# beltegeuse/rustlight

Measured on AMD Instinct MI355X. Metric: Msamples/s (paths/s) at 1080p x 128spp cbox, higher is better.
Workload: dtype f32

## Files before the change

rustlight_amd/csrc/device_types.h:

```cpp
#pragma once
#include <stdint.h>

namespace rl {

struct alignas(16) BvhNode {
    float lmin[3]; float lmax0;
    float lmax12[2]; float rmin01[2];
    float rmin2; float rmax[3];
    int32_t left, right; int32_t pad0, pad1;
};
static_assert(sizeof(BvhNode) == 64, "BvhNode must be 64 bytes");
static const int32_t RL_CHILD_NONE = (int32_t)0x80000000;

struct alignas(16) BvhNode2 {
    float lox[4], loy[4], loz[4];
    float hix[4], hiy[4], hiz[4];
    int32_t slot[4];
    int32_t child[2];
    int32_t pad[2];
};
static_assert(sizeof(BvhNode2) == 128, "BvhNode2 must be 128 bytes");

struct alignas(16) Bvh4Node {
    float org[3];
// ... 6 lines not shown
static_assert(sizeof(Bvh4Node) == 64, "Bvh4Node must be 64 bytes");

struct alignas(16) TriRecord {
    float v0[3]; float n0;
    float e1[3]; float n1;
    float e2[3]; float n2;
    float det;
    int32_t mesh;
    int32_t tri;
    int32_t gtri;
};
static_assert(sizeof(TriRecord) == 64, "TriRecord must be 64 bytes");

struct ColorTex {
    int32_t type;
    float c0[3];
    float c1[3];
    float offset[2];
    float scale[2];
    float line_width;
    int32_t bitmap;
    int32_t pad[3];
};
static_assert(sizeof(ColorTex) == 64, "ColorTex must be 64 bytes");

struct BitmapDesc { uint32_t w, h; uint64_t offset; };

struct Material {
    int32_t type;
    int32_t distribution;
    float exponent, weight_specular;
    float alpha_u, alpha_v;
    float glass_eta, glass_inv_eta;
    int32_t smooth;
    int32_t twosided;
    int32_t pad[2];
    ColorTex diffuse, specular, transmittance, eta, k;
};

struct MeshRecord {
    int32_t material;
    int32_t flags;
    float emission[3];
    float inv_area;
    float emitter_pdf;
    uint32_t vertex_base;
    uint32_t tri_base;
    uint32_t n_tris;
    uint32_t cdf_base;
    uint32_t ats_base;
    int32_t emission_type;
    float emission_scale;
    int32_t emission_bitmap;
};
enum { MESH_HAS_NORMALS = 1, MESH_HAS_UV = 2, MESH_IS_LIGHT = 4 };

enum { EMITTER_MESH = 0, EMITTER_ENV = 1, EMITTER_POINT = 2, EMITTER_DIRECTIONAL = 3 };
struct EmitterRecord {
    int32_t kind;
    int32_t mesh;
    float v[3];
    float c[3];
    float center[3];
    float radius;
    float pad[4];
};
static_assert(sizeof(EmitterRecord) == 64, "EmitterRecord must be 64 bytes");

struct LightNode {
    float bmin[3], bmax[3];
    float axis[3];
    float phi, cos_theta_o, cos_theta_e;
    int32_t left, right, parent;
    int32_t light;
};
static_assert(sizeof(LightNode) == 64, "LightNode must be 64 bytes");

struct CameraRecord {
    float sample_to_camera[16];
    float to_world[16];
    float position[3];
    uint32_t width, height;
};

struct MediumRecord {
    int32_t enabled;
    float sigma_a[3], sigma_s[3], sigma_t[3];
    int32_t phase;
    float g;
};

struct DeviceScene {
    const BvhNode* nodes;
    const TriRecord* tris;
    float root_min[3], root_max[3];
    int32_t root;
    uint32_t n_nodes, n_prims;
    uint32_t stack_depth;
    const BvhNode* nodes_t;
    int32_t root_t;
    const BvhNode2* nodes2;
    const Bvh4Node* nodes4;
    int32_t root4;
    uint32_t stack_depth4;
    const uint32_t* tri_indices;
    const float* positions;
    const float* normals;
    const float* uvs;
    const MeshRecord* meshes;
    const Material* materials;
    const BitmapDesc* bitmaps;
    const float* bitmap_texels;
    const EmitterRecord* emitters;
    const float* emitters_cdf;
    uint32_t n_emitters;
    int32_t env_emitter;
    float env_color[3];
    float env_pdf;
    uint32_t env_w, env_h;
    const float* env_texels;
    const float* env_cond_cdf;
    const float* env_cond_func;
    const float* env_marg_cdf;
    float env_marg_func_int;
    float env_sel_pdf;
    int32_t ats_root;
    const LightNode* ats_nodes;
    const int32_t* ats_light_mesh;
    const int32_t* ats_light_prim;
    const uint32_t* ats_leaf_of;
    const float* mesh_cdf;
    uint32_t n_meshes;
    CameraRecord camera;
    MediumRecord medium;
};

}
```

rustlight_amd/csrc/host/scene.cpp:

```cpp
#include "scene.h"
#include "../kernels/wavefront.h"
#include "../detmath_shared.h"

#include <algorithm>
#include <cmath>
#include <cstring>

namespace rl {

static const float kEpsilon = 0.0001f;
static const float kPi = 3.14159265358979323846f;

void build_cdf(const std::vector<float>& elements, std::vector<float>* cdf, float* func_int) {
    cdf->clear();
    cdf->reserve(elements.size() + 1);
    float cur = 0.0f;
    const float n = (float)elements.size();
    for (float e : elements) {
        cdf->push_back(cur);
        cur += e / n;
    }
    cdf->push_back(cur);
    if (cur != 0.0f)
        for (float& x : *cdf) x /= cur;
// ... 6 lines not shown
    t->type = d.type;
    for (int i = 0; i < 3; i++) { t->c0[i] = d.color0[i]; t->c1[i] = d.color1[i]; }
    for (int i = 0; i < 2; i++) { t->offset[i] = d.offset[i]; t->scale[i] = d.scale[i]; }
    t->line_width = d.line_width;
    t->bitmap = d.bitmap_id;
}

static Material convert_material(const rl_bsdf_desc& b) {
    Material m;
    std::memset(&m, 0, sizeof(m));
    m.type = b.type;
    m.distribution = b.distribution;
    m.exponent = b.exponent;
    m.weight_specular = b.weight_specular;
    m.alpha_u = b.alpha_u;
    m.alpha_v = b.alpha_v;
    m.glass_eta = b.glass_eta;
    m.glass_inv_eta = 1.0f / b.glass_eta;
    bool delta = false;
    switch (b.type) {
        case RL_BSDF_METAL: delta = b.distribution == RL_MICROFACET_NONE; break;
        case RL_BSDF_GLASS: delta = true; break;
        case RL_BSDF_SUBSTRATE: delta = b.distribution == RL_MICROFACET_NONE; break;
        default: break;
    }
    m.smooth = delta ? 1 : 0;
    m.twosided = b.type == RL_BSDF_GLASS ? 0 : 1;
    convert_color(b.diffuse, &m.diffuse);
    convert_color(b.specular, &m.specular);
    convert_color(b.transmittance, &m.transmittance);
    convert_color(b.eta, &m.eta);
    convert_color(b.k, &m.k);
    return m;
}

void flatten_scene(const rl_scene& scene, FlatScene* out) {
    *out = FlatScene();
    uint32_t vbase = 0, tbase = 0;
    for (size_t mi = 0; mi < scene.meshes.size(); mi++) {
        const HostMesh& m = scene.meshes[mi];
        MeshRecord r;
        std::memset(&r, 0, sizeof(r));
        r.material = (int32_t)out->materials.size();
        out->materials.push_back(convert_material(m.bsdf));
        r.flags = (m.normals.empty() ? 0 : MESH_HAS_NORMALS) | (m.uvs.empty() ? 0 : MESH_HAS_UV) | (m.is_light ? MESH_IS_LIGHT : 0);
        for (int i = 0; i < 3; i++) r.emission[i] = m.emission[i];
        r.emission_type = m.emission_type; r.emission_scale = m.emission_scale; r.emission_bitmap = m.emission_bitmap;
        r.inv_area = 1.0f / m.area_total();
        r.emitter_pdf = 0.0f;
        r.vertex_base = vbase;
        r.tri_base = tbase;
        r.n_tris = (uint32_t)m.n_tris();
        r.cdf_base = (uint32_t)out->mesh_cdf.size();
        out->mesh_tri_base.push_back(tbase);
        out->mesh_cdf.insert(out->mesh_cdf.end(), m.cdf.begin(), m.cdf.end());
        for (size_t v = 0; v < m.positions.size(); v++) {
            out->positions.push_back(m.positions[v].x); out->positions.push_back(m.positions[v].y); out->positions.push_back(m.positions[v].z);
            Vec3 n = m.normals.empty() ? Vec3{0, 0, 0} : m.normals[v];
            out->normals.push_back(n.x); out->normals.push_back(n.y); out->normals.push_back(n.z);
            out->uvs.push_back(m.uvs.empty() ? 0.0f : m.uvs[2 * v]);
            out->uvs.push_back(m.uvs.empty() ? 0.0f : m.uvs[2 * v + 1]);
        }
        for (uint32_t i : m.indices) out->tri_indices.push_back(i + vbase);
        vbase += (uint32_t)m.positions.size();
        tbase += (uint32_t)m.n_tris();
        out->meshes.push_back(r);
    }
    for (size_t e = 0; e < scene.emitters.size(); e++)
        if (scene.emitters[e].kind == EMITTER_MESH)
            out->meshes[scene.emitters[e].mesh].emitter_pdf = scene.emitters_cdf[e + 1] - scene.emitters_cdf[e];
    uint64_t off = 0;
    for (const HostBitmap& b : scene.bitmaps) {
        out->bitmaps.push_back({b.w, b.h, off});
        out->bitmap_texels.insert(out->bitmap_texels.end(), b.rgb.begin(), b.rgb.end());
        off += (uint64_t)b.w * b.h;
    }
}

}

using namespace rl;

bool rl_scene::rebuild_camera() {
    if (!to_world.inverse(&to_local)) return false;
    const float x_v = flip ? 1.0f : -1.0f;
    const float aspect = (float)width / (float)height;
    const float fov_rad = fov_axis == 0 ? fov_degrees * kPi / 180.0f : fov_degrees * aspect * kPi / 180.0f;
    camera_to_sample = Mat4::scale(-0.5f, -0.5f * aspect, 1.0f)
                                .times(Mat4::translate(-1.0f, -1.0f / aspect, 0.0f))
                                .times(perspective(fov_rad, 1.0f, 1e-2f, 1000.0f))
                                .times(Mat4::scale(x_v, 1.0f, -1.0f));
    if (!camera_to_sample.inverse(&sample_to_camera)) return false;
    cam_pos = to_world.xform_point({0.0f, 0.0f, 0.0f});
    has_camera = true;
    return true;
}

extern "C" {

int rl_scene_create(rl_scene** out) {
    if (!out) return RL_ERR_INVALID_ARGUMENT;
    *out = new rl_scene();
    return RL_OK;
}
void rl_scene_destroy(rl_scene* scene) { delete scene; }

// ... 372 lines not shown
```

rustlight_amd/csrc/host/scene.h:

```cpp
#pragma once
#include <cstdint>
#include <string>
#include <vector>

#include "../../../include/rustlight_amd.h"
#include "../device_types.h"
#include "hostmath.h"

namespace rl {

struct HostMesh {
    std::vector<Vec3> positions;
    std::vector<uint32_t> indices;
    std::vector<Vec3> normals;
    std::vector<float> uvs;
    rl_bsdf_desc bsdf;
    bool is_light = false;
    float emission[3] = {0, 0, 0};
    int emission_type = 0;
    float emission_scale = 1.0f;
    int emission_bitmap = -1;
    std::vector<float> cdf;
    float func_int = 0.0f;
    size_t n_tris() const { return indices.size() / 3; }
// ... 15 lines not shown
    rl::Vec3 cam_pos{0, 0, 0};
    std::vector<rl::HostMesh> meshes;
    std::vector<rl::HostBitmap> bitmaps;
    rl::MediumRecord medium{};
    bool emitters_built = false;
    std::vector<rl::EmitterRecord> other_emitters;
    bool has_env = false; float env_color[3] = {0, 0, 0};
    rl::HostBitmap env_map{0, 0, {}};
    std::vector<float> env_cond_cdf, env_cond_func, env_marg_cdf;
    float env_marg_func_int = 0.0f;
    std::vector<rl::EmitterRecord> emitters;
    std::vector<float> emitters_cdf;
    float bsphere_center[3] = {0, 0, 0};
    float bsphere_radius = 0;
    bool want_ats = false;
    int32_t ats_root = -1;
    std::vector<rl::LightNode> ats_nodes;
    std::vector<int32_t> ats_light_emitter, ats_light_prim;
    std::vector<uint32_t> ats_leaf_of;
    std::vector<uint32_t> ats_emitter_base;

    bool rebuild_camera();
};

namespace rl {

void build_cdf(const std::vector<float>& elements, std::vector<float>* cdf, float* func_int);

struct BvhBuild {
    std::vector<BvhNode> nodes;
    std::vector<TriRecord> tris;
    float root_min[3], root_max[3];
    int32_t root = RL_CHILD_NONE;
    uint32_t stack_depth = 1;
    std::vector<float> ref_boxes;
    std::vector<uint64_t> ref_info, ref_count;
    std::vector<int32_t> ref_prim_mesh, ref_prim_tri;
};
void build_bvh(const rl_scene& scene, BvhBuild* out);
void treelet_blocks(const BvhBuild& bvh, std::vector<BvhNode>* nodes_out, int32_t* root_out);
void two_level_nodes(const BvhBuild& bvh, std::vector<BvhNode2>* out, uint64_t* stats3 = nullptr);
struct Bvh4Build { std::vector<Bvh4Node> nodes; int32_t root = RL_CHILD_NONE; uint32_t stack_depth = 1; };
void build_bvh4(const BvhBuild& bvh, Bvh4Build* out);

struct FlatScene {
    std::vector<uint32_t> tri_indices;
    std::vector<float> positions, normals, uvs;
    std::vector<MeshRecord> meshes;
    std::vector<Material> materials;
    std::vector<BitmapDesc> bitmaps;
    std::vector<float> bitmap_texels;
    std::vector<float> mesh_cdf;
    std::vector<uint32_t> mesh_tri_base;
};
void flatten_scene(const rl_scene& scene, FlatScene* out);

int build_light_tree(rl_scene* scene, std::string* err);
int host_math_sweep(int fn, uint32_t first_bits, uint32_t stride, uint32_t period, size_t n, const float* b, size_t n_b, int swap, float* out);
int read_pfm(const char* path, uint32_t* w, uint32_t* h, std::vector<float>* rgb);
int load_pbrt(const char* path, bool use_shading_normals, rl_scene** out, std::string* err);

}
```

rustlight_amd/csrc/kernels/shading.hip.h:

```cpp
#pragma once
#include "../device_types.h"
#include "devmath.hip.h"

namespace rl {

enum { BSDF_DIFFUSE = 0, BSDF_PHONG = 1, BSDF_METAL = 2, BSDF_GLASS = 3, BSDF_SUBSTRATE = 4 };
enum { TEXTURE_CONSTANT = 0, TEXTURE_CHECKER = 1, TEXTURE_GRID = 2, TEXTURE_BITMAP = 3 };
enum { MICRO_NONE = 0, MICRO_BECKMANN = 1, MICRO_GGX = 2 };
enum { PDF_SOLID_ANGLE = 0, PDF_AREA = 1, PDF_DISCRETE = 2 };

struct SurfacePoint {
    V3 p, n_g, n_s, wi;
    Frame frame;
    V2 uv;
    bool has_uv;
    int mesh;
};

RL_DEV unsigned long long f32_as_usize(float f) { if (!(f > 0.0f)) return 0ull; if (f >= 1.8446744e19f) return ~0ull; return (unsigned long long)f; }
RL_DEV int f32_as_i32(float f) { if (f != f) return 0; if (f >= 2147483648.0f) return 2147483647; if (f <= -2147483648.0f) return (-2147483647 - 1); return (int)f; }
RL_DEV float modulo1(float a) { return fmodf(fmodf(a, 1.0f) + 1.0f, 1.0f); }

RL_DEV Col tex_color(const DeviceScene& sc, const ColorTex& t, bool has_uv, V2 uv) {
    if (t.type == TEXTURE_CONSTANT) return mkc(t.c0[0], t.c0[1], t.c0[2]);
// ... 401 lines not shown
    unsigned long long x = f32_as_usize(ux * (float)sc.env_w), y = f32_as_usize(uy * (float)sc.env_h);
    unsigned long long i = (unsigned long long)sc.env_w * y + x;
    if (i >= (unsigned long long)sc.env_w * sc.env_h) return czero();
    return mkc(sc.env_texels[3 * i], sc.env_texels[3 * i + 1], sc.env_texels[3 * i + 2]);
}
RL_DEV float env_direct_pdf(const DeviceScene& sc, V3 d) {
    if (sc.env_w == 0u) return sc.env_pdf;
    V2 uv = env_to_spherical(d);
    float p = env_bin_pdf(sc, f32_as_usize(uv.x * (float)sc.env_w), f32_as_usize(uv.y * (float)sc.env_h));
    float st = m_sinf(kPi * uv.y);
    float v = st == 0.0f ? 0.0f : div_rn(p, (2.0f * powi_f(kPi, 2)) * st);
    return v * sc.env_sel_pdf;
}
RL_DEV void env_sample_direction(const DeviceScene& sc, V2 u, V3* d, Col* value, float* pdf) {
    float y = cdf_sample_continuous(sc.env_marg_cdf, sc.env_h, u.y);
    unsigned long long row = f32_as_usize(y);
    float x = cdf_sample_continuous(sc.env_cond_cdf + row * (sc.env_w + 1u), sc.env_w, u.x);
    x = clamp_f(x, 0.0f, (float)sc.env_w - 1.0f);
    y = clamp_f(y, 0.0f, (float)sc.env_h - 1.0f);
    unsigned long long px = f32_as_usize(x), py = f32_as_usize(y);
    const float* t = sc.env_texels + 3ull * (py * sc.env_w + px);
    float p = env_bin_pdf(sc, px, py);
    float sp, cp, st, ct;
    m_sincosf(div_rn(2.0f * kPi, (float)sc.env_w) * x, &sp, &cp);
    m_sincosf(div_rn(kPi, (float)sc.env_h) * y, &st, &ct);
    *d = mk3(st * cp, st * sp, ct);
    if (st == 0.0f) { *value = czero(); *pdf = 0.0f; }
    else { *value = mkc(t[0], t[1], t[2]); *pdf = div_rn(p, (2.0f * powi_f(kPi, 2)) * st); }
}

RL_DEV bool bsphere_intersect(V3 center, float radius, V3 o, V3 d, float tnear, float tfar, float* t_out) {
    V3 d_p = center - o;
    float a = length2(d);
    float b = 2.0f * dot(d_p, d);
    float c = length2(d_p) - radius * radius;
    float x0, x1;
    if (a == 0.0f) {
        if (b == 0.0f) return false;
        float v = div_rn(-c, b);
        x0 = v; x1 = v;
    } else {
        float disc = b * b - 4.0f * a * c;
        if (disc < 0.0f) return false;
        float d_sqrt = sqrt_rn(disc);
        float tmp = b < 0.0f ? -0.5f * (b - d_sqrt) : -0.5f * (b + d_sqrt);
        float r0 = div_rn(tmp, a), r1 = div_rn(c, tmp);
        if (r0 > r1) { x0 = r1; x1 = r0; } else { x0 = r0; x1 = r1; }
    }
    if (x0 < tnear) { if (x1 < tfar) { *t_out = x1; return true; } return false; }
    if (x0 < tfar) { *t_out = x0; return true; }
    return false;
}

template <int LIGHTS = LIGHTS_ANY>
RL_DEV void mesh_sample_triangle(const DeviceScene& sc, const MeshRecord& mr, unsigned int prim, float pdf_area, V3 p, V2 uv, LightSample* ls) {
    unsigned int gtri = mr.tri_base + prim;
    unsigned int i0 = sc.tri_indices[3 * gtri], i1 = sc.tri_indices[3 * gtri + 1], i2 = sc.tri_indices[3 * gtri + 2];
    V3 v0 = mk3(sc.positions[3 * i0], sc.positions[3 * i0 + 1], sc.positions[3 * i0 + 2]);
    V3 v1 = mk3(sc.positions[3 * i1], sc.positions[3 * i1 + 1], sc.positions[3 * i1 + 2]);
    V3 v2 = mk3(sc.positions[3 * i2], sc.positions[3 * i2 + 1], sc.positions[3 * i2 + 2]);
    V2 b = uniform_sample_triangle(uv);
    float w2 = 1.0f - b.x - b.y;
    V3 pos = v0 * b.x + v1 * b.y + v2 * w2;
    V3 n_g = normalize(cross(v2 - v0, v1 - v0));
    if (mr.flags & MESH_HAS_NORMALS) {
        V3 n0 = mk3(sc.normals[3 * i0], sc.normals[3 * i0 + 1], sc.normals[3 * i0 + 2]);
        V3 n1 = mk3(sc.normals[3 * i1], sc.normals[3 * i1 + 1], sc.normals[3 * i1 + 2]);
        V3 n2 = mk3(sc.normals[3 * i2], sc.normals[3 * i2 + 1], sc.normals[3 * i2 + 2]);
        V3 n = n0 * b.x + n1 * b.y + n2 * w2;
        float nl = length2(n);
        if (nl == 0.0f) n = n_g;
        else if (nl != 1.0f) n = n / sqrt_rn(nl);
        if (dot(n_g, n) < 0.0f) n_g = -n_g;
    }
    if (pdf_area < 0.0f) pdf_area = div_rn(1.0f, length(cross(v1 - v0, v2 - v0)) * 0.5f);
    V3 d = pos - p;
    float dist = length(d);
    if (dist != 0.0f) d = d / dist;
    float geom = dist != 0.0f ? div_rn(rmax(dot(n_g, -d), 0.0f), dist * dist) : 0.0f;
    float pdf = geom == 0.0f ? 0.0f : div_rn(pdf_area, geom);
    Col emit;
    if (LIGHTS == LIGHTS_AREA_ONLY || __builtin_expect(mr.emission_type == 0, 1)) emit = mkc(mr.emission[0], mr.emission[1], mr.emission[2]);
    else emit = mesh_emit_sampled(sc.bitmaps, sc.bitmap_texels, sc.uvs, mr.emission_type, mr.emission_scale, mr.emission_bitmap, (mr.flags & MESH_HAS_UV) != 0, i0, i1, i2, b.x, b.y, w2);
    ls->weight = pdf == 0.0f ? czero() : emit * geom / pdf_area;
    ls->pdf = pdf; ls->pdf_kind = PDF_SOLID_ANGLE;
    ls->p = pos; ls->n = n_g; ls->d = d;
}

RL_DEV float ats_cos_subtended(V3 bmin, V3 bmax, V3 p) {
    V3 c = (bmax - bmin) * 0.5f + bmin;
    float radius = length(c - bmax);
    if (length2(p - c) < radius * radius) return -1.0f;
    float sin2 = div_rn(radius * radius, length2(c - p));
    return sqrt_rn(rmax(1.0f - sin2, 0.0f));
}
RL_DEV float ats_cos_sub(float sa, float ca, float sb, float cb) { return ca > cb ? 1.0f : ca * cb + sa * sb; }
RL_DEV float ats_sin_sub(float sa, float ca, float sb, float cb) { return ca > cb ? 1.0f : sa * cb - ca * sb; }
RL_DEV float ats_importance(const LightNode& nd, V3 p, bool has_n, V3 n) {
    V3 bmin = mk3(nd.bmin[0], nd.bmin[1], nd.bmin[2]), bmax = mk3(nd.bmax[0], nd.bmax[1], nd.bmax[2]);
    V3 pc = (bmax - bmin) * 0.5f + bmin;
    float d2 = rmax(length2(p - pc), 0.0001f);
    V3 wi = normalize(p - pc);
    float cos_theta = dot(mk3(nd.axis[0], nd.axis[1], nd.axis[2]), wi);
    float sin_theta = sqrt_rn(rmax(1.0f - cos_theta * cos_theta, 0.0f));
    float cos_u = ats_cos_subtended(bmin, bmax, p);
    float sin_u = sqrt_rn(rmax(1.0f - cos_u * cos_u, 0.0f));
    float sin_o = sqrt_rn(rmax(1.0f - nd.cos_theta_o * nd.cos_theta_o, 0.0f));
    float cos_x = ats_cos_sub(sin_theta, cos_theta, sin_o, nd.cos_theta_o);
    float sin_x = ats_sin_sub(sin_theta, cos_theta, sin_o, nd.cos_theta_o);
    float cos_p = ats_cos_sub(sin_x, cos_x, sin_u, cos_u);
    if (cos_p <= nd.cos_theta_e) return 0.0f;
    float imp = div_rn(nd.phi * cos_p, d2);
    if (has_n) {
        float cos_i = fabsf(dot(wi, n));
        float sin_i = sqrt_rn(rmax(1.0f - cos_i * cos_i, 0.0f));
        imp = imp * ats_cos_sub(sin_i, cos_i, sin_u, cos_u);
    }
// ... 159 lines not shown
```

rustlight_amd/csrc/kernels/trace.hip.h:

```cpp
#pragma once
#include "../device_types.h"
#include "devmath.hip.h"
#include <type_traits>

namespace rl {

struct Hit { float t, u, v; int prim; int steps = 0, tris = 0, fetches = 0; };

#ifndef RL_LDS_NODE_STRIDE
#define RL_LDS_NODE_STRIDE 17
#endif
#ifndef RL_LDS_TRI_STRIDE4
#define RL_LDS_TRI_STRIDE4 5
#endif
static constexpr int kLdsNodeStride = RL_LDS_NODE_STRIDE;
static constexpr int kLdsTriStride4 = RL_LDS_TRI_STRIDE4;
RL_DEV __host__ unsigned lds_nodes_float4s(unsigned n_nodes) { return (n_nodes * (unsigned)kLdsNodeStride + 3u) / 4u; }
RL_DEV __host__ unsigned lds_scene_float4s(unsigned n_nodes, unsigned n_prims) { return lds_nodes_float4s(n_nodes) + n_prims * (unsigned)kLdsTriStride4; }

RL_DEV bool slab(V3 lo, V3 hi, V3 o, V3 inv_d, float tnear, float tfar, float* t_entry) {
    const float x0 = (lo.x - o.x) * inv_d.x, x1 = (hi.x - o.x) * inv_d.x;
    const float y0 = (lo.y - o.y) * inv_d.y, y1 = (hi.y - o.y) * inv_d.y;
    const float z0 = (lo.z - o.z) * inv_d.z, z1 = (hi.z - o.z) * inv_d.z;
    const bool sx = inv_d.x < 0.0f, sy = inv_d.y < 0.0f, sz = inv_d.z < 0.0f;
// ... 21 lines not shown
        const V3 pv = (o + t * d) - v0;
        const V3 u0 = cross(e1, pv);
        const V3 w0 = cross(pv, e2);
        const bool facing = !(dot(u0, n) < 0.0f) & !(dot(w0, n) < 0.0f);
        const float uu = dot(u0, u0), ww = dot(w0, w0);
#if defined(RL_FAST_MATH)
        accept = facing & (det > 0.0f) & (__builtin_amdgcn_sqrtf(uu) + __builtin_amdgcn_sqrtf(ww) <= det);
#else
        const float s = __builtin_amdgcn_sqrtf(uu) + __builtin_amdgcn_sqrtf(ww);
        const bool in_range = __builtin_fminf(__builtin_fminf(uu, ww), det) >= 0x1p-100f;
        const bool sure_in = in_range & (s <= det * 0.99999f), sure_out = in_range & (s >= det * 1.00001f);
        accept = facing & sure_in;
        if (facing & !sure_in & !sure_out) {
            const float v = div_rn(sqrt_rn(uu), det);
            const float u = div_rn(sqrt_rn(ww), det);
            accept = !(u < 0.0f || v < 0.0f || u > 1.0f || v > 1.0f) && (u + v <= 1.0f);
        }
#endif
    }
    hit.t = accept ? t : hit.t;
    hit.prim = accept ? prim : hit.prim;
    return accept;
}

struct SceneRecs {
    const float4* nodes;
    const float4* tris;
};

struct NodeFetchLds;
struct NodeFetchGlobal;
template <bool LDS_ONLY>
struct TravStackT {
    using NodeFetch = typename std::conditional<LDS_ONLY, NodeFetchLds, NodeFetchGlobal>::type;
    static constexpr bool kLdsOnly = LDS_ONLY;
#ifdef RL_FAST_MATH
    static constexpr bool kBvh4 = !LDS_ONLY;
#else
    static constexpr bool kBvh4 = false;
#endif
    static constexpr bool kTwoLevel = false;
    static constexpr int kTriStride4 = LDS_ONLY ? kLdsTriStride4 : 4;
    static constexpr int kNodeRefScale = LDS_ONLY ? 4 * kLdsNodeStride : 1;
    static constexpr int lds_stride = 256;
    typedef int i2v __attribute__((ext_vector_type(2)));
    typedef __attribute__((address_space(3))) i2v LdsPair;
    typedef __attribute__((address_space(1))) i2v GlobPair;
    using LdsPtr = typename std::conditional<kBvh4, int2*, LdsPair*>::type;
    using GlobPtr = typename std::conditional<kBvh4, int*, GlobPair*>::type;
    LdsPtr lds; int lds_levels;
    GlobPtr glob; size_t glob_stride;
    RL_DEV void push(int sp, int code, float dist, bool counts = true) const { push_to(lds, glob, sp, code, dist, counts); }
    RL_DEV void get(int sp, int* code, float* dist) const { get_from(lds, glob, sp, code, dist); }
    RL_DEV void push_to(LdsPair* l, GlobPair* g, int sp, int code, float dist, bool counts) const {
        i2v e; e.x = code; e.y = __float_as_int(dist);
        if (LDS_ONLY || sp < lds_levels) l[sp * lds_stride] = e;
        else if (counts) g[(size_t)(sp - lds_levels) * glob_stride] = e;
    }
    RL_DEV void get_from(const LdsPair* l, const GlobPair* g, int sp, int* code, float* dist) const {
        i2v e;
        if (LDS_ONLY || sp < lds_levels) e = l[sp * lds_stride];
        else e = g[(size_t)(sp - lds_levels) * glob_stride];
        *code = e.x; *dist = __int_as_float(e.y);
    }
    RL_DEV void push_to(int2* l, int* g, int sp, int code, float dist, bool) const {
        if (sp < lds_levels) l[sp * lds_stride] = make_int2(code, __float_as_int(dist));
        else { size_t k = (size_t)(2 * (sp - lds_levels)); g[k * glob_stride] = code; g[(k + 1) * glob_stride] = __float_as_int(dist); }
    }
    RL_DEV void get_from(const int2* l, const int* g, int sp, int* code, float* dist) const {
        if (sp < lds_levels) { const int2 e = l[sp * lds_stride]; *code = e.x; *dist = __int_as_float(e.y); }
        else { size_t k = (size_t)(2 * (sp - lds_levels)); *code = g[k * glob_stride]; *dist = __int_as_float(g[(k + 1) * glob_stride]); }
    }
};
using TravStack = TravStackT<false>;
struct TravStack2 : TravStackT<false> {
    static constexpr bool kTwoLevel = true;
    static constexpr bool kBvh4 = false;
    RL_DEV explicit TravStack2(const TravStackT<false>& s) : TravStackT<false>(s) {}
};

typedef float f4v __attribute__((ext_vector_type(4)));
typedef const f4v __attribute__((address_space(4))) F4c;
struct NodePlanes { float lnx, lny, lnz, lfx, lfy, lfz, rnx, rny, rnz, rfx, rfy, rfz; int id1, id2; };

struct NodeFetchLds {
    static constexpr bool kHasUniform = false;
    RL_DEV NodePlanes uniform(int) const { return NodePlanes(); }
    const float *nx, *ny, *nz, *fx, *fy, *fz; const int* ids;
    RL_DEV NodeFetchLds(const SceneRecs& recs, V3 inv_d) {
        const float* b = reinterpret_cast<const float*>(recs.nodes);
        const bool sx = inv_d.x < 0.0f, sy = inv_d.y < 0.0f, sz = inv_d.z < 0.0f;
        nx = b + (sx ? 3 : 0); fx = b + (sx ? 0 : 3);
        ny = b + (sy ? 4 : 1); fy = b + (sy ? 1 : 4);
        nz = b + (sz ? 5 : 2); fz = b + (sz ? 2 : 5);
        ids = reinterpret_cast<const int*>(b) + 12;
    }
    RL_DEV NodePlanes operator()(int cur) const {
        NodePlanes p;
#define RL_AT(ptr, off) (*reinterpret_cast<const float*>(reinterpret_cast<const char*>(ptr) + cur + 4 * (off)))
        p.lnx = RL_AT(nx, 0); p.rnx = RL_AT(nx, 6); p.lny = RL_AT(ny, 0); p.rny = RL_AT(ny, 6); p.lnz = RL_AT(nz, 0); p.rnz = RL_AT(nz, 6);
        p.lfx = RL_AT(fx, 0); p.rfx = RL_AT(fx, 6); p.lfy = RL_AT(fy, 0); p.rfy = RL_AT(fy, 6); p.lfz = RL_AT(fz, 0); p.rfz = RL_AT(fz, 6);
        p.id1 = __float_as_int(RL_AT(ids, 0)); p.id2 = __float_as_int(RL_AT(ids, 1));
#undef RL_AT
        return p;
    }
};
// ... 2 lines not shown
    RL_DEV NodeFetchGlobal(const SceneRecs& recs, V3 inv_d) : nodes(recs.nodes), sx(inv_d.x < 0.0f), sy(inv_d.y < 0.0f), sz(inv_d.z < 0.0f) {}
    RL_DEV NodePlanes operator()(int cur) const {
        const float4* q = nodes + 4 * cur;
        const float4 a = q[0], b = q[1], c = q[2];
        const float4 e = q[3];
        NodePlanes p;
        p.lnx = sx ? a.w : a.x; p.lfx = sx ? a.x : a.w; p.lny = sy ? b.x : a.y; p.lfy = sy ? a.y : b.x; p.lnz = sz ? b.y : a.z; p.lfz = sz ? a.z : b.y;
        p.rnx = sx ? c.y : b.z; p.rfx = sx ? b.z : c.y; p.rny = sy ? c.z : b.w; p.rfy = sy ? b.w : c.z; p.rnz = sz ? c.w : c.x; p.rfz = sz ? c.x : c.w;
        p.id1 = __float_as_int(e.x); p.id2 = __float_as_int(e.y);
        return p;
    }
    static constexpr bool kHasUniform = true;
    RL_DEV NodePlanes uniform(int cur) const {
        const F4c* q = (const F4c*)(nodes) + 4 * cur;
        const f4v a = q[0], b = q[1], c = q[2], e = q[3];
        NodePlanes p;
        p.lnx = sx ? a.w : a.x; p.lfx = sx ? a.x : a.w; p.lny = sy ? b.x : a.y; p.lfy = sy ? a.y : b.x; p.lnz = sz ? b.y : a.z; p.lfz = sz ? a.z : b.y;
        p.rnx = sx ? c.y : b.z; p.rfx = sx ? b.z : c.y; p.rny = sy ? c.z : b.w; p.rfy = sy ? b.w : c.z; p.rnz = sz ? c.w : c.x; p.rfz = sz ? c.x : c.w;
        p.id1 = __float_as_int(e.x); p.id2 = __float_as_int(e.y);
        return p;
    }
};

#ifndef RL_VOTE_NUM
#define RL_VOTE_NUM 3
#define RL_VOTE_DEN 2
#endif
#ifndef RL_VOTE4_NUM
#define RL_VOTE4_NUM 3
#define RL_VOTE4_DEN 2
#endif
template <bool ANY_HIT, class Stack>
RL_DEV bool traverse4(const SceneRecs& recs, int root, V3 root_lo, V3 root_hi, V3 o, V3 d, float tnear, float tfar, Hit& hit, const Stack& st);
template <bool ANY_HIT, class Stack>
RL_DEV bool traverse2(const SceneRecs& recs, int root, V3 root_lo, V3 root_hi, V3 o, V3 d, float tnear, float tfar, Hit& hit, const Stack& st);
template <class Stack>
RL_DEV const float4* streamed_nodes(const DeviceScene& sc) {
    return Stack::kBvh4 ? reinterpret_cast<const float4*>(sc.nodes4) : (Stack::kTwoLevel ? reinterpret_cast<const float4*>(sc.nodes2) : reinterpret_cast<const float4*>(sc.nodes));
}

template <bool ANY_HIT, class Stack>
RL_DEV bool traverse(const SceneRecs& recs, int root, V3 root_lo, V3 root_hi, V3 o, V3 d, float tnear, float tfar,
                     Hit& hit, const Stack& st) {
    if constexpr (Stack::kBvh4) return traverse4<ANY_HIT>(recs, root, root_lo, root_hi, o, d, tnear, tfar, hit, st);
    if constexpr (Stack::kTwoLevel) return traverse2<ANY_HIT>(recs, root, root_lo, root_hi, o, d, tnear, tfar, hit, st);
    V3 inv_d = mk3(div_rn(1.0f, d.x), div_rn(1.0f, d.y), div_rn(1.0f, d.z));
    float dummy;
    int cur = root >= 0 ? root * Stack::kNodeRefScale : root;
    if (!slab(root_lo, root_hi, o, inv_d, tnear, tfar, &dummy)) cur = RL_CHILD_NONE;
    int sp = 0;
    bool found = false;
    typename Stack::NodeFetch fetch(recs, inv_d);
    constexpr int kPop = -1;
    auto node_trip = [&]() {
        if (cur >= 0) {
            hit.steps++;
            NodePlanes p;
            const int cur0 = __builtin_amdgcn_readfirstlane(cur);
            if (Stack::NodeFetch::kHasUniform && __ballot(cur != cur0) == 0ull) p = fetch.uniform(cur0);
            else p = fetch(cur);
            const float d1 = __builtin_fmaxf(__builtin_fmaxf(__builtin_fmaxf((p.lnx - o.x) * inv_d.x, (p.lny - o.y) * inv_d.y), (p.lnz - o.z) * inv_d.z), tnear);
            const float f1 = __builtin_fminf(__builtin_fminf(__builtin_fminf((p.lfx - o.x) * inv_d.x, (p.lfy - o.y) * inv_d.y), (p.lfz - o.z) * inv_d.z), hit.t);
            const float d2 = __builtin_fmaxf(__builtin_fmaxf(__builtin_fmaxf((p.rnx - o.x) * inv_d.x, (p.rny - o.y) * inv_d.y), (p.rnz - o.z) * inv_d.z), tnear);
            const float f2 = __builtin_fminf(__builtin_fminf(__builtin_fminf((p.rfx - o.x) * inv_d.x, (p.rfy - o.y) * inv_d.y), (p.rfz - o.z) * inv_d.z), hit.t);
            const bool v1 = !(f1 <= d1), v2 = !(f2 <= d2);
            const bool right_first = v2 & (!v1 | (d1 > d2));
            st.push(sp, right_first ? p.id1 : p.id2, right_first ? d1 : d2, v1 && v2);
            sp += (v1 && v2) ? 1 : 0;
            cur = (v1 || v2) ? (right_first ? p.id2 : p.id1) : kPop;
        }
        if (cur == kPop) {
            cur = RL_CHILD_NONE;
            if (sp > 0) {
                sp--;
                int code; float dist;
                st.get(sp, &code, &dist);
                cur = dist < hit.t ? code : kPop;
            }
        }
    };
    auto leaf_visit = [&]() -> bool {
        const unsigned int code = (unsigned int)(~cur);
        const int first = (int)(code >> 2), count = (int)(code & 3u);
        bool uni = false;
        if (Stack::NodeFetch::kHasUniform) uni = __ballot(cur != __builtin_amdgcn_readfirstlane(cur)) == 0ull;
        for (int k = 0; k < count; k++) {
            hit.tris++;
            float4 q0, q1, q2, q3;
            if (uni) {
                const F4c* q = (const F4c*)(recs.tris) + 4 * (__builtin_amdgcn_readfirstlane(first) + k);
                const f4v a = q[0], b = q[1], c = q[2], e = q[3];
                q0 = make_float4(a.x, a.y, a.z, a.w); q1 = make_float4(b.x, b.y, b.z, b.w); q2 = make_float4(c.x, c.y, c.z, c.w); q3 = make_float4(e.x, e.y, e.z, e.w);
            } else {
                const float4* q = recs.tris + Stack::kTriStride4 * (first + k);
                q0 = q[0]; q1 = q[1]; q2 = q[2]; q3 = q[3];
            }
            if (tri_test(q0, q1, q2, q3, o, d, hit, first + k)) {
                found = true;
                if (ANY_HIT) return true;
            }
        }
        cur = kPop;
        return false;
    };
    if (Stack::kLdsOnly) {
        while (cur != RL_CHILD_NONE) {
            while (cur >= 0 || cur == kPop) node_trip();
            if (cur != RL_CHILD_NONE && leaf_visit()) return true;
        }
    } else {
#if defined(RL_TRAVERSE_SPARSE)
        while (cur != RL_CHILD_NONE) {
            if (cur >= 0 || cur == kPop) node_trip();
            else if (leaf_visit()) return true;
        }
#else
        for (;;) {
            const bool in_node = cur >= 0 || cur == kPop;
            const bool in_leaf = !in_node && cur != RL_CHILD_NONE;
            const int n_node = __popcll(__ballot(in_node)), n_leaf = __popcll(__ballot(in_leaf));
            if (n_node + n_leaf == 0) break;
            if (n_node > 0 && n_node * RL_VOTE_DEN >= RL_VOTE_NUM * n_leaf) { if (in_node) node_trip(); }
            else if (in_leaf && leaf_visit()) return true;
        }
#endif
    }
    if (!ANY_HIT && found) {
        const float4* q = recs.tris + Stack::kTriStride4 * hit.prim;
        tri_uv(q[0], q[1], q[2], q[3], o, d, hit.t, &hit.u, &hit.v);
    }
// ... 448 lines not shown
```

rustlight_amd/csrc/kernels/wavefront.hip:

```cpp
#include <hip/hip_runtime.h>

#include <algorithm>
#include <atomic>
#include <chrono>
#include <cmath>
#include <cstdio>
#include <cstring>
#include <memory>
#include <string>
#include <thread>
#include <vector>

#include "common.hip.h"
#include "rngjump.h"
#include "../host/hip_buffer.h"
#include "../host/photontree.h"
#include "../host/beamtree.h"
#include "phototree.h"
#include "../host/scene.h"
#include "wavefront.h"
#include "knobs.h"
#include "light.hip.h"

namespace rl {
// ... 109 lines not shown
template <bool LDS_SCENE>
__global__ void __launch_bounds__(256) k_shadow(RenderConst rc, DeviceScene sc, Pool pool, StackConf stc) { trace_kernel_body<LDS_SCENE, true>(sc, pool, stc); }

__global__ void __launch_bounds__(256) k_trace_batch(DeviceScene sc, StackConf stc, unsigned n, const float* o, const float* d, float* t_out, float* u_out,
                                                     float* v_out, int* mesh_out, int* tri_out) {
    extern __shared__ __attribute__((aligned(16))) float4 smem[];
    SceneRecs recs;
    recs.nodes = streamed_nodes<TravStackT<false>>(sc);
    recs.tris = reinterpret_cast<const float4*>(sc.tris);
    unsigned i = blockIdx.x * blockDim.x + threadIdx.x;
    const TravStack stack = make_stack(stc, reinterpret_cast<unsigned*>(smem), i);
    if (i >= n) return;
    V3 ro = mk3(o[3 * i], o[3 * i + 1], o[3 * i + 2]), rd = mk3(d[3 * i], d[3 * i + 1], d[3 * i + 2]);
    Hit hit;
    trace_closest(sc, recs, stack, ro, rd, hit);
    t_out[i] = hit.t; u_out[i] = hit.u; v_out[i] = hit.v;
    if (hit.prim >= 0) { mesh_out[i] = sc.tris[hit.prim].mesh; tri_out[i] = sc.tris[hit.prim].tri; }
    else { mesh_out[i] = -1; tri_out[i] = -1; }
}

__global__ void __launch_bounds__(256) k_trace_batch_two_level(DeviceScene sc, StackConf stc, unsigned n, const float* o, const float* d, float* t_out, float* u_out,
                                                               float* v_out, int* mesh_out, int* tri_out, int* steps_out, int any_hit) {
    extern __shared__ __attribute__((aligned(16))) float4 smem[];
    SceneRecs recs;
    recs.nodes = reinterpret_cast<const float4*>(sc.nodes2);
    recs.tris = reinterpret_cast<const float4*>(sc.tris);
    unsigned i = blockIdx.x * blockDim.x + threadIdx.x;
    const TravStack2 stack(make_stack(stc, reinterpret_cast<unsigned*>(smem), i));
    if (i >= n) return;
    V3 ro = mk3(o[3 * i], o[3 * i + 1], o[3 * i + 2]), rd = mk3(d[3 * i], d[3 * i + 1], d[3 * i + 2]);
    Hit hit; hit.t = kF32Max; hit.u = 0.0f; hit.v = 0.0f; hit.prim = -1;
    if (any_hit) {
        hit.t = t_out[i];
        const bool f = traverse<true>(recs, sc.root, mk3(sc.root_min[0], sc.root_min[1], sc.root_min[2]), mk3(sc.root_max[0], sc.root_max[1], sc.root_max[2]), ro, rd, kEps, hit.t, hit, stack);
        t_out[i] = f ? 1.0f : 0.0f; steps_out[i] = hit.steps;
        return;
    }
    trace_closest(sc, recs, stack, ro, rd, hit);
    t_out[i] = hit.t; u_out[i] = hit.u; v_out[i] = hit.v; steps_out[i] = hit.steps;
    if (hit.prim >= 0) { mesh_out[i] = sc.tris[hit.prim].mesh; tri_out[i] = sc.tris[hit.prim].tri; }
    else { mesh_out[i] = -1; tri_out[i] = -1; }
}

__global__ void __launch_bounds__(256) k_visible_batch(DeviceScene sc, StackConf stc, unsigned n, const float* p0a, const float* p1a, unsigned char* out) {
    extern __shared__ __attribute__((aligned(16))) float4 smem[];
    SceneRecs recs;
    recs.nodes = streamed_nodes<TravStackT<false>>(sc);
    recs.tris = reinterpret_cast<const float4*>(sc.tris);
    unsigned i = blockIdx.x * blockDim.x + threadIdx.x;
    const TravStack stack = make_stack(stc, reinterpret_cast<unsigned*>(smem), i);
    if (i >= n) return;
    V3 p0 = mk3(p0a[3 * i], p0a[3 * i + 1], p0a[3 * i + 2]), p1 = mk3(p1a[3 * i], p1a[3 * i + 1], p1a[3 * i + 2]);
    out[i] = shadow_visible(sc, recs, stack, p0, p1) ? 1 : 0;
}

__global__ void k_numerics_probe(unsigned n, const float* a, const float* b, float* out_div, float* out_sqrt, float* out_mad, float* out_sin,
                                 float* out_cos, float* out_exp, float* out_log, float* out_pow, float* out_acos, float* out_atan2) {
    unsigned i = blockIdx.x * blockDim.x + threadIdx.x;
    if (i >= n) return;
    out_div[i] = div_rn(a[i], b[i]);
    out_sqrt[i] = sqrt_rn(fabsf(a[i]));
    out_mad[i] = a[i] * b[i] + a[i];
    out_sin[i] = dm::sinf_det(a[i]);
    out_cos[i] = dm::cosf_det(a[i]);
    out_exp[i] = dm::expf_det(a[i]);
    out_log[i] = dm::logf_det(fabsf(a[i]));
    out_pow[i] = dm::powf_det(fabsf(a[i]), b[i]);
    out_acos[i] = dm::acosf_det(a[i] * 0.15f);
    out_atan2[i] = dm::atan2f_det(a[i], b[i]);
}

__global__ void k_math_sweep(int fn, int swap, unsigned first_bits, unsigned stride, unsigned period, unsigned n, const float* b, float b_const, float* out) {
    unsigned i = blockIdx.x * blockDim.x + threadIdx.x;
    if (i >= n) return;
    const float g = __uint_as_float(first_bits + (period ? i % period : i) * stride);
    const float c = b ? b[i] : b_const;
    const float x = swap ? c : g, y = swap ? g : c;
    float r;
    switch (fn) {
        case RL_MATH_SINF: r = dm::sinf_det(x); break;
        case RL_MATH_COSF: r = dm::cosf_det(x); break;
        case RL_MATH_EXPF: r = dm::expf_det(x); break;
        case RL_MATH_LOGF: r = dm::logf_det(x); break;
        case RL_MATH_POWF: r = dm::powf_det(x, y); break;
        case RL_MATH_ACOSF: r = dm::acosf_det(x); break;
        case RL_MATH_ATAN2F: r = dm::atan2f_det(x, y); break;
        case RL_MATH_ASINF: r = dm::asinf_det(x); break;
        case RL_MATH_SQRT_RN: r = sqrt_rn(x); break;
        case RL_MATH_DIV_RN: r = div_rn(x, y); break;
        default: r = x * y + x; break;
    }
    out[i] = r;
}

}

using namespace rl;

static thread_local std::string g_last_error;
void rl_set_error(const std::string& s) { g_last_error = s; }
extern "C" const char* rl_last_error(void) { return g_last_error.c_str(); }

struct rl_context {
    int device = 0;
    hipStream_t stream = nullptr;
    DeviceScene ds{};
// ... 106 lines not shown
        DeviceScene& ds = ctx->ds;
        if ((rc = upload(ctx, bvh.nodes, &ds.nodes)) != RL_OK) break;
        if ((rc = upload(ctx, bvh.tris, &ds.tris)) != RL_OK) break;
        for (int i = 0; i < 3; i++) { ds.root_min[i] = bvh.root_min[i]; ds.root_max[i] = bvh.root_max[i]; }
        ds.root = bvh.root;
        ds.n_nodes = (uint32_t)bvh.nodes.size();
        ds.n_prims = (uint32_t)bvh.tris.size();
        ds.stack_depth = bvh.stack_depth;
        ds.nodes4 = nullptr; ds.root4 = RL_CHILD_NONE; ds.stack_depth4 = 0;
        ds.nodes_t = nullptr; ds.root_t = RL_CHILD_NONE;
        ds.nodes2 = nullptr;
        if ((rc = upload(ctx, flat.tri_indices, &ds.tri_indices)) != RL_OK) break;
        if ((rc = upload(ctx, flat.positions, &ds.positions)) != RL_OK) break;
        if ((rc = upload(ctx, flat.normals, &ds.normals)) != RL_OK) break;
        if ((rc = upload(ctx, flat.uvs, &ds.uvs)) != RL_OK) break;
        for (MeshRecord& mr : flat.meshes) mr.ats_base = 0xffffffffu;
        std::vector<int32_t> ats_light_mesh;
        if (scene->ats_root >= 0) {
            for (size_t e = 0; e < scene->emitters.size(); e++) flat.meshes[scene->emitters[e].mesh].ats_base = scene->ats_emitter_base[e];
            for (int32_t e : scene->ats_light_emitter) ats_light_mesh.push_back(scene->emitters[e].mesh);
        }
        if ((rc = upload(ctx, flat.meshes, &ds.meshes)) != RL_OK) break;
        ds.ats_root = scene->ats_root;
        if ((rc = upload(ctx, scene->ats_nodes, &ds.ats_nodes)) != RL_OK) break;
        if ((rc = upload(ctx, ats_light_mesh, &ds.ats_light_mesh)) != RL_OK) break;
        if ((rc = upload(ctx, scene->ats_light_prim, &ds.ats_light_prim)) != RL_OK) break;
        if ((rc = upload(ctx, scene->ats_leaf_of, &ds.ats_leaf_of)) != RL_OK) break;
        if ((rc = upload(ctx, flat.materials, &ds.materials)) != RL_OK) break;
        if ((rc = upload(ctx, flat.bitmaps, &ds.bitmaps)) != RL_OK) break;
        if ((rc = upload(ctx, flat.bitmap_texels, &ds.bitmap_texels)) != RL_OK) break;
        if ((rc = upload(ctx, scene->emitters, &ds.emitters)) != RL_OK) break;
        if ((rc = upload(ctx, scene->emitters_cdf, &ds.emitters_cdf)) != RL_OK) break;
        ds.n_emitters = (uint32_t)scene->emitters.size();
        ds.env_emitter = -1;
        for (size_t e = 0; e < scene->emitters.size(); e++)
            if (scene->emitters[e].kind == EMITTER_ENV) {
                ds.env_emitter = (int32_t)e;
                for (int k = 0; k < 3; k++) ds.env_color[k] = scene->emitters[e].c[k];
                ds.env_pdf = (1.0f / (3.14159265358979323846f * 4.0f)) * (scene->emitters_cdf[e + 1] - scene->emitters_cdf[e]);
                ds.env_sel_pdf = scene->emitters_cdf[e + 1] - scene->emitters_cdf[e];
            }
        ds.env_w = ds.env_h = 0;
        if (ds.env_emitter >= 0 && scene->env_map.w) {
            ds.env_w = scene->env_map.w; ds.env_h = scene->env_map.h;
            ds.env_marg_func_int = scene->env_marg_func_int;
            if ((rc = upload(ctx, scene->env_map.rgb, &ds.env_texels)) != RL_OK) break;
            if ((rc = upload(ctx, scene->env_cond_cdf, &ds.env_cond_cdf)) != RL_OK) break;
            if ((rc = upload(ctx, scene->env_cond_func, &ds.env_cond_func)) != RL_OK) break;
            if ((rc = upload(ctx, scene->env_marg_cdf, &ds.env_marg_cdf)) != RL_OK) break;
        }
        if (ds.env_emitter >= 0 && scene->medium.enabled) { rl_set_error("an environment emitter cannot be combined with a medium (paths/edge.rs:94)"); rc = RL_ERR_UNSUPPORTED; break; }
        if ((rc = upload(ctx, flat.mesh_cdf, &ds.mesh_cdf)) != RL_OK) break;
        ds.n_meshes = (uint32_t)flat.meshes.size();
        scene->sample_to_camera.to_cols(ds.camera.sample_to_camera);
        scene->to_world.to_cols(ds.camera.to_world);
        ds.camera.position[0] = scene->cam_pos.x; ds.camera.position[1] = scene->cam_pos.y; ds.camera.position[2] = scene->cam_pos.z;
        ds.camera.width = scene->width; ds.camera.height = scene->height;
        {
            scene->camera_to_sample.to_cols(ctx->light_cam.camera_to_sample);
            scene->to_local.to_cols(ctx->light_cam.to_local);
            const Vec3 p0 = scene->sample_to_camera.xform_point({0.0f, 0.0f, 0.0f}), p1 = scene->sample_to_camera.xform_point({1.0f, 1.0f, 0.0f});
            const float zmin = std::fmin(p0.z, p1.z), zmax = std::fmax(p0.z, p1.z);
            ctx->light_cam.rect_min[0] = std::fmin(p0.x, p1.x) / zmin; ctx->light_cam.rect_min[1] = std::fmin(p0.y, p1.y) / zmin;
            ctx->light_cam.rect_max[0] = std::fmax(p0.x, p1.x) / zmax; ctx->light_cam.rect_max[1] = std::fmax(p0.y, p1.y) / zmax;
        }
        ds.medium = scene->medium;
        {
            const char* why = "";
            if ((ctx->rect_lights_rc = build_rect_lights(*scene, &ctx->rect_lights, &why)) != RL_OK) ctx->rect_lights_err = why;
        }
        ctx->area_lights_only = scene->ats_root < 0 && !ctx->knobs.has(K_GENERIC_LIGHTS);
        for (const EmitterRecord& e : scene->emitters) if (e.kind != EMITTER_MESH) ctx->area_lights_only = false;
        for (const EmitterRecord& e : scene->emitters) if (e.kind == EMITTER_DIRECTIONAL) ctx->has_directional = true;
        for (const HostMesh& hm : scene->meshes) if (hm.is_light && hm.emission_type != RL_EMISSION_COLOR) ctx->area_lights_only = false;
        ctx->single_bsdf = true;
        ctx->bsdf_type = flat.materials.empty() ? 0 : flat.materials[0].type;
        for (const Material& m : flat.materials) if (m.type != ctx->bsdf_type) ctx->single_bsdf = false;
        ctx->scene_lds_bytes = (size_t)16 * lds_scene_float4s(ds.n_nodes, ds.n_prims);
        ctx->lds_scene = ctx->scene_lds_bytes <= 48 * 1024 && ds.stack_depth <= (uint32_t)kLdsStackLevels;
        {
            int lds_limit = 64 * 1024;
            if (hipDeviceGetAttribute(&lds_limit, hipDeviceAttributeMaxSharedMemoryPerBlock, device) != hipSuccess) { (void)hipGetLastError(); lds_limit = 64 * 1024; }
            ctx->lds_limit = (size_t)std::max(lds_limit, 16 * 1024);
            const size_t worst = ctx->scene_lds_bytes + std::max<size_t>(272 * sizeof(unsigned), kFusedColdBytes) + (size_t)2 * kLdsStackLevels * 256 * sizeof(int);
            if (worst > (size_t)lds_limit) ctx->lds_scene = false;
        }
        if (ctx->knobs.has(K_FORCE_STREAMING)) ctx->lds_scene = false;
        if (!ctx->lds_scene) {
            Bvh4Build b4;
            build_bvh4(bvh, &b4);
            if ((rc = upload(ctx, b4.nodes, &ds.nodes4)) != RL_OK) break;
            ds.root4 = b4.root; ds.stack_depth4 = b4.stack_depth;
            std::vector<BvhNode> blocks;
            int32_t root_t = RL_CHILD_NONE;
            treelet_blocks(bvh, &blocks, &root_t);
            if ((rc = upload(ctx, blocks, &ds.nodes_t)) != RL_OK) break;
            ds.root_t = root_t;
        }
        if (ctx->d_counters.ensure(1) != RL_OK) { rl_set_error("hipMalloc counters"); rc = RL_ERR_HIP; break; }
        if (ctx->h_counters.ensure(1) != RL_OK) { rl_set_error("hipHostMalloc counters"); rc = RL_ERR_HIP; break; }
    } while (0);
    if (rc != RL_OK) { rl_context_destroy(ctx); return rc; }
    *out = ctx;
    return RL_OK;
}

// ... 923 lines not shown
```

Baseline: 5505.

## Precompute packed light triangle records and drop distances from any-hit LDS stack

Adds a per-light-triangle 64-byte record holding vertex positions, the precomputed geometric normal and the vertex indices, built on the device at scene load. Light sampling then reads three or four float4 loads instead of an index gather, three position gathers and a cross/normalize. Separately, any-hit traversal with an LDS-only stack now pushes and pops only the node code and skips the stored entry distance, so pops no longer cull against hit.t. The risks are extra memory, setup work at scene load, and possibly more node visits in shadow rays.

```diff
diff --git a/rustlight_amd/csrc/device_types.h b/rustlight_amd/csrc/device_types.h
--- a/rustlight_amd/csrc/device_types.h
+++ b/rustlight_amd/csrc/device_types.h
@@ -82,8 +82,19 @@
     int32_t emission_type;
     float emission_scale;
     int32_t emission_bitmap;
+    uint32_t light_base;
 };
+static_assert(sizeof(MeshRecord) == 64, "MeshRecord must be 64 bytes");
 enum { MESH_HAS_NORMALS = 1, MESH_HAS_UV = 2, MESH_IS_LIGHT = 4 };
+
+struct alignas(16) LightTri {
+    float v0[3]; float n0;
+    float v1[3]; float n1;
+    float v2[3]; float n2;
+    uint32_t idx[3];
+    uint32_t pad;
+};
+static_assert(sizeof(LightTri) == 64, "LightTri must be 64 bytes");
 
 enum { EMITTER_MESH = 0, EMITTER_ENV = 1, EMITTER_POINT = 2, EMITTER_DIRECTIONAL = 3 };
 struct EmitterRecord {
@@ -161,6 +172,7 @@
     const uint32_t* ats_leaf_of;
     const float* mesh_cdf;
     uint32_t n_meshes;
+    const LightTri* light_tris;
     CameraRecord camera;
     MediumRecord medium;
 };
diff --git a/rustlight_amd/csrc/host/scene.cpp b/rustlight_amd/csrc/host/scene.cpp
--- a/rustlight_amd/csrc/host/scene.cpp
+++ b/rustlight_amd/csrc/host/scene.cpp
@@ -82,6 +82,8 @@
         r.tri_base = tbase;
         r.n_tris = (uint32_t)m.n_tris();
         r.cdf_base = (uint32_t)out->mesh_cdf.size();
+        r.light_base = out->n_light_tris;
+        if (m.is_light) out->n_light_tris += (uint32_t)m.n_tris();
         out->mesh_tri_base.push_back(tbase);
         out->mesh_cdf.insert(out->mesh_cdf.end(), m.cdf.begin(), m.cdf.end());
         for (size_t v = 0; v < m.positions.size(); v++) {
diff --git a/rustlight_amd/csrc/host/scene.h b/rustlight_amd/csrc/host/scene.h
--- a/rustlight_amd/csrc/host/scene.h
+++ b/rustlight_amd/csrc/host/scene.h
@@ -91,6 +91,7 @@
     std::vector<float> bitmap_texels;
     std::vector<float> mesh_cdf;
     std::vector<uint32_t> mesh_tri_base;
+    uint32_t n_light_tris = 0;
 };
 void flatten_scene(const rl_scene& scene, FlatScene* out);
 
diff --git a/rustlight_amd/csrc/kernels/shading.hip.h b/rustlight_amd/csrc/kernels/shading.hip.h
--- a/rustlight_amd/csrc/kernels/shading.hip.h
+++ b/rustlight_amd/csrc/kernels/shading.hip.h
@@ -477,17 +477,34 @@
     return false;
 }
 
-template <int LIGHTS = LIGHTS_ANY>
-RL_DEV void mesh_sample_triangle(const DeviceScene& sc, const MeshRecord& mr, unsigned int prim, float pdf_area, V3 p, V2 uv, LightSample* ls) {
-    unsigned int gtri = mr.tri_base + prim;
+RL_DEV LightTri light_tri_record(const DeviceScene& sc, unsigned int gtri) {
     unsigned int i0 = sc.tri_indices[3 * gtri], i1 = sc.tri_indices[3 * gtri + 1], i2 = sc.tri_indices[3 * gtri + 2];
     V3 v0 = mk3(sc.positions[3 * i0], sc.positions[3 * i0 + 1], sc.positions[3 * i0 + 2]);
     V3 v1 = mk3(sc.positions[3 * i1], sc.positions[3 * i1 + 1], sc.positions[3 * i1 + 2]);
     V3 v2 = mk3(sc.positions[3 * i2], sc.positions[3 * i2 + 1], sc.positions[3 * i2 + 2]);
+    V3 n_g = normalize(cross(v2 - v0, v1 - v0));
+    LightTri r;
+    r.v0[0] = v0.x; r.v0[1] = v0.y; r.v0[2] = v0.z; r.n0 = n_g.x;
+    r.v1[0] = v1.x; r.v1[1] = v1.y; r.v1[2] = v1.z; r.n1 = n_g.y;
+    r.v2[0] = v2.x; r.v2[1] = v2.y; r.v2[2] = v2.z; r.n2 = n_g.z;
+    r.idx[0] = i0; r.idx[1] = i1; r.idx[2] = i2; r.pad = 0u;
+    return r;
+}
+
+template <int LIGHTS = LIGHTS_ANY>
+RL_DEV void mesh_sample_triangle(const DeviceScene& sc, const MeshRecord& mr, unsigned int prim, float pdf_area, V3 p, V2 uv, LightSample* ls) {
+    const float4* lt = reinterpret_cast<const float4*>(sc.light_tris) + 4 * (size_t)(mr.light_base + prim);
+    const float4 l0 = lt[0], l1 = lt[1], l2 = lt[2];
+    V3 v0 = mk3(l0.x, l0.y, l0.z), v1 = mk3(l1.x, l1.y, l1.z), v2 = mk3(l2.x, l2.y, l2.z);
     V2 b = uniform_sample_triangle(uv);
     float w2 = 1.0f - b.x - b.y;
     V3 pos = v0 * b.x + v1 * b.y + v2 * w2;
-    V3 n_g = normalize(cross(v2 - v0, v1 - v0));
+    V3 n_g = mk3(l0.w, l1.w, l2.w);
+    unsigned int i0 = 0u, i1 = 0u, i2 = 0u;
+    if ((mr.flags & MESH_HAS_NORMALS) || (LIGHTS != LIGHTS_AREA_ONLY && mr.emission_type != 0)) {
+        const float4 l3 = lt[3];
+        i0 = __float_as_uint(l3.x); i1 = __float_as_uint(l3.y); i2 = __float_as_uint(l3.z);
+    }
     if (mr.flags & MESH_HAS_NORMALS) {
         V3 n0 = mk3(sc.normals[3 * i0], sc.normals[3 * i0 + 1], sc.normals[3 * i0 + 2]);
         V3 n1 = mk3(sc.normals[3 * i1], sc.normals[3 * i1 + 1], sc.normals[3 * i1 + 2]);
diff --git a/rustlight_amd/csrc/kernels/trace.hip.h b/rustlight_amd/csrc/kernels/trace.hip.h
--- a/rustlight_amd/csrc/kernels/trace.hip.h
+++ b/rustlight_amd/csrc/kernels/trace.hip.h
@@ -97,6 +97,9 @@
     GlobPtr glob; size_t glob_stride;
     RL_DEV void push(int sp, int code, float dist, bool counts = true) const { push_to(lds, glob, sp, code, dist, counts); }
     RL_DEV void get(int sp, int* code, float* dist) const { get_from(lds, glob, sp, code, dist); }
+    typedef __attribute__((address_space(3))) int LdsWord;
+    RL_DEV void push_code(int sp, int code) const { *reinterpret_cast<LdsWord*>(lds + sp * lds_stride) = code; }
+    RL_DEV int get_code(int sp) const { return *reinterpret_cast<const LdsWord*>(lds + sp * lds_stride); }
     RL_DEV void push_to(LdsPair* l, GlobPair* g, int sp, int code, float dist, bool counts) const {
         i2v e; e.x = code; e.y = __float_as_int(dist);
         if (LDS_ONLY || sp < lds_levels) l[sp * lds_stride] = e;
@@ -205,6 +208,7 @@
     bool found = false;
     typename Stack::NodeFetch fetch(recs, inv_d);
     constexpr int kPop = -1;
+    constexpr bool kCodeOnly = ANY_HIT && Stack::kLdsOnly;
     auto node_trip = [&]() {
         if (cur >= 0) {
             hit.steps++;
@@ -218,7 +222,8 @@
             const float f2 = __builtin_fminf(__builtin_fminf(__builtin_fminf((p.rfx - o.x) * inv_d.x, (p.rfy - o.y) * inv_d.y), (p.rfz - o.z) * inv_d.z), hit.t);
             const bool v1 = !(f1 <= d1), v2 = !(f2 <= d2);
             const bool right_first = v2 & (!v1 | (d1 > d2));
-            st.push(sp, right_first ? p.id1 : p.id2, right_first ? d1 : d2, v1 && v2);
+            if constexpr (kCodeOnly) st.push_code(sp, right_first ? p.id1 : p.id2);
+            else st.push(sp, right_first ? p.id1 : p.id2, right_first ? d1 : d2, v1 && v2);
             sp += (v1 && v2) ? 1 : 0;
             cur = (v1 || v2) ? (right_first ? p.id2 : p.id1) : kPop;
         }
@@ -226,9 +231,12 @@
             cur = RL_CHILD_NONE;
             if (sp > 0) {
                 sp--;
-                int code; float dist;
-                st.get(sp, &code, &dist);
-                cur = dist < hit.t ? code : kPop;
+                if constexpr (kCodeOnly) cur = st.get_code(sp);
+                else {
+                    int code; float dist;
+                    st.get(sp, &code, &dist);
+                    cur = dist < hit.t ? code : kPop;
+                }
             }
         }
     };
diff --git a/rustlight_amd/csrc/kernels/wavefront.hip b/rustlight_amd/csrc/kernels/wavefront.hip
--- a/rustlight_amd/csrc/kernels/wavefront.hip
+++ b/rustlight_amd/csrc/kernels/wavefront.hip
@@ -185,6 +185,13 @@
     if (i >= n) return;
     V3 p0 = mk3(p0a[3 * i], p0a[3 * i + 1], p0a[3 * i + 2]), p1 = mk3(p1a[3 * i], p1a[3 * i + 1], p1a[3 * i + 2]);
     out[i] = shadow_visible(sc, recs, stack, p0, p1) ? 1 : 0;
+}
+
+__global__ void __launch_bounds__(256) k_light_records(DeviceScene sc, unsigned mesh, unsigned n_records, LightTri* out) {
+    const MeshRecord mr = sc.meshes[mesh];
+    const unsigned i = blockIdx.x * blockDim.x + threadIdx.x;
+    if (i >= mr.n_tris || mr.light_base + i >= n_records) return;
+    out[mr.light_base + i] = light_tri_record(sc, mr.tri_base + i);
 }
 
 __global__ void k_numerics_probe(unsigned n, const float* a, const float* b, float* out_div, float* out_sqrt, float* out_mad, float* out_sin,
@@ -397,6 +404,18 @@
         if (ds.env_emitter >= 0 && scene->medium.enabled) { rl_set_error("an environment emitter cannot be combined with a medium (paths/edge.rs:94)"); rc = RL_ERR_UNSUPPORTED; break; }
         if ((rc = upload(ctx, flat.mesh_cdf, &ds.mesh_cdf)) != RL_OK) break;
         ds.n_meshes = (uint32_t)flat.meshes.size();
+        {
+            if ((rc = upload(ctx, std::vector<LightTri>(flat.n_light_tris), &ds.light_tris)) != RL_OK) break;
+            LightTri* records = const_cast<LightTri*>(ds.light_tris);
+            bool ok = true;
+            for (size_t m = 0; m < flat.meshes.size() && ok; m++) {
+                const MeshRecord& mr = flat.meshes[m];
+                if (!(mr.flags & MESH_IS_LIGHT) || mr.n_tris == 0) continue;
+                hipLaunchKernelGGL(k_light_records, dim3((mr.n_tris + 255u) / 256u), dim3(256), 0, ctx->stream, ds, (unsigned)m, flat.n_light_tris, records);
+                ok = hipGetLastError() == hipSuccess;
+            }
+            if (!ok || hipStreamSynchronize(ctx->stream) != hipSuccess) { (void)hipGetLastError(); rl_set_error("k_light_records failed"); rc = RL_ERR_HIP; break; }
+        }
         scene->sample_to_camera.to_cols(ds.camera.sample_to_camera);
         scene->to_world.to_cols(ds.camera.to_world);
         ds.camera.position[0] = scene->cam_pos.x; ds.camera.position[1] = scene->cam_pos.y; ds.camera.position[2] = scene->cam_pos.z;
```

New measurement: 5551, median of 6. About the same (+0.8%).
